# NumericalEarth/Breeze.jl

Measured on AMD Instinct MI355X. Metric: grid-cells advanced/sec (tendency+Poisson step), 512^3 anelastic, higher is better.
Workload: dtype f64

## Files before the change

breeze.jl_amd/csrc/bz_tendency5_kernels.h:

```cpp
#pragma once
#include "bz_internal.h"
#include "bz_weno.h"
#include "bz_tendency4_kernels.h"

typedef long long ix_t;
typedef unsigned ix32_t;

struct LevRow5 {
    double rho, rrho;
    double rho_f, rrho_f;
    double Ax, Ay, Vinv_c;
    double pi;
    double Vinv_f, T_r;
    double pad[6];
};
struct Lev5 {
    const LevRow5 *p;
#ifdef __HIPCC__
    __device__ __forceinline__ double at(int k, int f) const { return ((ColPtr::cptr)(const double *)p)[(long long)k * 16 + f]; }
    __device__ __forceinline__ double rho(int k) const { return at(k, 0); }
    __device__ __forceinline__ double rrho(int k) const { return at(k, 1); }
    __device__ __forceinline__ double rho_f(int k) const { return at(k, 2); }
    __device__ __forceinline__ double rrho_f(int k) const { return at(k, 3); }
    __device__ __forceinline__ double Ax(int k) const { return at(k, 4); }
    __device__ __forceinline__ double Ay(int k) const { return at(k, 5); }
    __device__ __forceinline__ double Vinv_c(int k) const { return at(k, 6); }
    __device__ __forceinline__ double pi(int k) const { return at(k, 7); }
    __device__ __forceinline__ double Vinv_f(int k) const { return at(k, 8); }
    __device__ __forceinline__ double T_r(int k) const { return at(k, 9); }
#endif
};
static_assert(sizeof(LevRow5) == 16 * sizeof(double), "LevRow5 is sixteen reals");

#define BZ_LEAN_WAVES (sizeof(double) == 8 ? 4 : 6)
#define BZ5_SCALAR_WAVES (sizeof(double) == 8 ? 4 : 6)
#define BZ6_W_WAVES 4
constexpr int BZ5_EB = 64;

struct Lean5 {
    const double *ru, *rv, *rw;
    const double *pa, *pb;
    double *out;
    double *oa, *ob;
    double *T;
    ColPtr pi_dry;
    const LevRow5 *lev;
    int mforce;
    double cor_f;
    ColPtr Fu, Fv;
    ColPtr Su, Sv;
    const double *vel, *bT, *bq;
    const int *qstate;
    int xcd;
    int by0, bys;
};
// ... 33 lines not shown
    const double th = bz_cdiv(rth, rho, rrho), q = bz_cdiv(rq, rho, rrho);
    if (pi_dry.p && __all(q == 0.0)) return pi_dry[k] * th;
    const double qd = 1.0 - q;
    const double cpm = qd * g.cpd + q * g.cpv;
    return bz_exner_factor(g, k, q, cpm) * th;
}

__device__ __forceinline__ double bz_temperature5r(const DevGrid &g, double rth, double rq, int k, double rho, double rrho, double pi)
{
    const double th = bz_cdiv(rth, rho, rrho), q = bz_cdiv(rq, rho, rrho);
    if (__all(q == 0.0)) return pi * th;
    const double qd = 1.0 - q;
    const double cpm = qd * g.cpd + q * g.cpv;
    return bz_exner_factor(g, k, q, cpm) * th;
}

template <bool WY> __device__ __forceinline__ int by5_face(const DevGrid &g, int j) { return WY ? bz_buffer_face(j, g.Ny) : 3; }
template <bool WY> __device__ __forceinline__ int by5_center(const DevGrid &g, int j) { return WY ? bz_buffer_center(j, g.Ny) : 3; }
template <bool WY>
__device__ __forceinline__ double bz_up5y(double m3, double m2, double m1, double p0, double p1, double p2, bool left, int B)
{
    if constexpr (WY) return bz_upB(m3, m2, m1, p0, p1, p2, left, B);
    else return bz_up5(m3, m2, m1, p0, p1, p2, left);
}
template <bool WY>
__device__ __forceinline__ double bz_symm4y(double qm2, double qm1, double q0, double qp1, int B)
{
    if constexpr (WY) return (B == 3) ? bz_symm4(qm2, qm1, q0, qp1) : bz_symm2(qm1, q0);
    else return bz_symm4(qm2, qm1, q0, qp1);
}

template <int TY, bool WY, bool DRYQ>
__device__ __forceinline__ void k5_scalar_pair_body(const DevGrid &g, const Lean5 &F, int kchunk, const RKEpilogue &E, double *Tp, double *FYp, int *ZF)
{
    constexpr bool Q = !DRYQ;
    constexpr int TR = TY + 6, TC = 72;
    constexpr int NHALO = TR * 70 - TY * 64;
    constexpr int NT = 64 * TY;
    constexpr int HPT = (NHALO + NT - 1) / NT;
    double(*T)[2][TR][TC] = (double(*)[2][TR][TC])Tp;
    double(*FY)[2][TY + 1][64] = (double(*)[2][TY + 1][64])FYp;
    constexpr bool ZS = Q;

    int bx, by, bz;
    bz_block5(F, bx, by, bz);
    const int tx = threadIdx.x, ty = threadIdx.y, t = ty * 64 + tx;
// ... 245 lines not shown
    }
}


template <bool DRYQ, bool GUARD>
__device__ __forceinline__ bool bz_lean_skip(const Lean5 &F)
{
    if constexpr (!GUARD) return false;
    const bool dry = F.qstate != nullptr && __builtin_amdgcn_readfirstlane(*F.qstate) == 1;
    return dry != DRYQ;
}
template <int TY, bool WY = false, bool DRYQ = false, bool GUARD = true>
__global__ __launch_bounds__(64 * TY) __attribute__((amdgpu_waves_per_eu(BZ5_SCALAR_WAVES, BZ5_SCALAR_WAVES))) void k5_scalar_pair(DevGrid g, Lean5 F, int kchunk, RKEpilogue E)
{
    constexpr int TR = TY + 6, TC = 72;
    __shared__ double T[2 * 2 * TR * TC];
    __shared__ double FY[2 * 2 * (TY + 1) * 64];
    __shared__ int ZF[3];
    if (bz_lean_skip<DRYQ, GUARD>(F)) return;
    k5_scalar_pair_body<TY, WY, DRYQ>(g, F, kchunk, E, T, FY, ZF);
}

template <int KIND>
__device__ __forceinline__ double flux_x_lean(const DevGrid &g, const Tend3Fields &F, const double *__restrict__ m, int i, int j, int k, int By = 3)
{
    const long long n = g.idx(i, j, k);
    const double a = (KIND == T3_V && By != 3) ? bz_symm2(g.Ax[k] * F.ru[n - g.Sx], g.Ax[k] * F.ru[n]) : adv_x<KIND>(g, F, n, k);
    const double rh = (KIND == T3_W) ? g.rho_f[k] : g.rho[k], rr = (KIND == T3_W) ? g.rrho_f[k] : g.rrho[k];
    if constexpr (KIND == T3_U)
        return a * bz_up5(bz_cdiv(m[n - 2], rh, rr), bz_cdiv(m[n - 1], rh, rr), bz_cdiv(m[n], rh, rr), bz_cdiv(m[n + 1], rh, rr),
                          bz_cdiv(m[n + 2], rh, rr), bz_cdiv(m[n + 3], rh, rr), a > 0.0);
    else
        return a * bz_up5(bz_cdiv(m[n - 3], rh, rr), bz_cdiv(m[n - 2], rh, rr), bz_cdiv(m[n - 1], rh, rr), bz_cdiv(m[n], rh, rr),
                          bz_cdiv(m[n + 1], rh, rr), bz_cdiv(m[n + 2], rh, rr), a > 0.0);
}


template <int TY, bool MF = false, bool WY = false, bool ST = false>
__global__ __launch_bounds__(64 * TY, BZ_LEAN_WAVES) void k6_u(DevGrid g, Lean5 L, int kchunk, RKEpilogue E)
{
    static_assert(!(ST && WY), "stored-velocity instantiations: periodic / slab rows");
    constexpr int TR = TY + 6, TC = 72, NT = 64 * TY;
    constexpr int NH1 = TR * 70 - TY * 64;
    constexpr int NH2 = 3 * (TY + 1) + 64 + 3 * TY;
    static_assert(NH1 <= NT && NH2 <= NT, "one frame cell of each kind per thread");
    __shared__ double U[2][TR][TC];
    __shared__ double RU[2][TY][TC];
    __shared__ double RV[2][TY + 1][TC];
    __shared__ double RW[2][TY][TC];
    __shared__ double FY[2][TY + 1][64];
    int bx, by, bz;
    bz_block5(L, bx, by, bz);
    const int tx = threadIdx.x, ty = threadIdx.y, t = ty * 64 + tx, tc = tx + 3;
    const int i0 = bx * 64, j0 = by * TY;
    const int i = i0 + tx, j = j0 + ty;
    const int ic = min(i, g.Nx + 2), jc = min(j, g.Ny + 2);
    const int ie = i0 - 1, le = 0;
    const int kbeg = bz * kchunk, kend = min(kbeg + kchunk, g.Nz);
    if (kbeg >= kend) return;
    const ix_t sz = (ix_t)g.Sxy;
    const bool store = (i < g.Nx) && (j < g.Ny);
    const double *__restrict__ ru = L.ru, *__restrict__ rv = L.rv, *__restrict__ rw = L.rw;
    const double *__restrict__ vel = ST ? L.vel : L.ru;
    Tend3Fields F;
    F.ru = L.ru; F.rv = L.rv; F.rw = L.rw; F.u = F.v = F.w = F.T = F.q = nullptr; F.c = ST ? L.vel : nullptr; F.G = L.out;
    ix_t n = (ix_t)g.idx(ic, jc, kbeg);
    const bool h1ok = t < NH1;
    int h1r = 0, h1c = 0;
    {
        const int h = h1ok ? t : 0;
        if (h < 6 * 70) { const int rr = h / 70; h1c = h - rr * 70; h1r = (rr < 3) ? rr : TY + rr; }
        else { const int hh = h - 6 * 70, rr = hh / 6, cc = hh - rr * 6; h1r = 3 + rr; h1c = (cc < 3) ? cc : 64 + cc; }
    }
    const ix_t h1n = (ix_t)g.idx(min(i0 - 3 + h1c, g.Nx + 2), min(j0 - 3 + h1r, g.Ny + 2), kbeg);
    const bool h1raw = h1ok && h1r >= 3 && h1r < TY + 3 && (h1c == 2 || h1c == 67 || h1c == 68);
    const bool h2ok = t < NH2;
    int h2sel = 0, h2r = 0, h2c = 0;
    {
        const int id = h2ok ? t : 0;
        if (id < 3 * (TY + 1)) { h2r = id / 3; const int cc = id - 3 * h2r; h2c = (cc < 2) ? 1 + cc : 67; }
        else if (id < 3 * (TY + 1) + 64) { h2r = TY; h2c = 3 + (id - 3 * (TY + 1)); }
        else { h2sel = 1; const int m = id - 3 * (TY + 1) - 64; h2r = m / 3; const int cc = m - 3 * h2r; h2c = (cc < 2) ? 1 + cc : 67; }
    }
    const double *__restrict__ h2src = h2sel ? rw : rv;
    const ix_t h2n = (ix_t)g.idx(min(i0 - 3 + h2c, g.Nx + 2), min(j0 + h2r, g.Ny + 2), kbeg) + (h2sel ? sz : (ix_t)0);

    double r[6];
#pragma unroll
    for (int s = 0; s < 6; ++s) r[s] = ST ? vel[n + s * sz - 3 * sz] : bz_cdiv(ru[n + s * sz - 3 * sz], g.rho[kbeg + s - 3], g.rrho[kbeg + s - 3]);
    double fz_lo = vflux<T3_U>(g, F, n, kbeg, r[0], r[1], r[2], r[3], r[4], r[5]);
    double q0 = ru[n], q1 = ru[n + sz], q2 = ru[n + 2 * sz];
    U[0][ty + 3][tc] = r[3];
    RU[0][ty][tc] = q0;
    RV[0][ty][tc] = rv[n];
    RW[0][ty][tc] = rw[n + sz];
    if (h1ok) {
        const double raw = (ST && !h1raw) ? 0.0 : ru[h1n];
        U[0][h1r][h1c] = ST ? vel[h1n] : bz_cdiv(raw, g.rho[kbeg], g.rrho[kbeg]);
        if (h1raw) RU[0][h1r - 3][h1c] = raw;
    }
    if (h2ok) { if (h2sel) RW[0][h2r][h2c] = h2src[h2n]; else RV[0][h2r][h2c] = h2src[h2n]; }
    double tcur_raw = ru[n + 3 * sz];
    double tcur_v = ST ? vel[n + 3 * sz] : 0.0;
    double u0cur = (E.mode == 2) ? E.u0[n] : 0.0;
    __syncthreads();

    double edge = 0.0;
    int buf = 0;
    for (int k = kbeg; k < kend; ++k, n += sz) {
        const ix_t lev1 = (ix_t)(k + 1 - kbeg) * sz;
        const double p_top = ST ? ru[n + sz] : ru[n + ((k + 4 <= g.Nz + g.Hz - 1) ? 4 * sz : 3 * sz)];
        const double p_topv = ST ? vel[n + ((k + 4 <= g.Nz + g.Hz - 1) ? 4 * sz : 3 * sz)] : 0.0;
        const double p_h1 = h1ok ? (ST ? vel : ru)[h1n + lev1] : 0.0;
        const double p_h1raw = (ST && h1raw) ? ru[h1n + lev1] : 0.0;
        const double p_h2 = h2ok ? h2src[h2n + lev1] : 0.0;
        const double p_rv = rv[n + sz], p_rw = rw[n + 2 * sz];
        const double p_u0 = (E.mode == 2) ? E.u0[n + sz] : 0.0;
        if (((k - kbeg) & (BZ5_EB - 1)) == 0) {
            const int kk = min(k + (tx & (BZ5_EB - 1)), kend - 1);
            edge = ST ? flux_x_at<T3_U>(g, F, ie, jc, kk) : flux_x_lean<T3_U>(g, F, ru, ie, jc, kk);
        }
        const int src = (k - kbeg) & (BZ5_EB - 1);
        const double Ax = g.Ax[k], Ay = g.Ay[k], Az = g.Az;
        const double c0 = r[3];
        const double(*Uk)[TC] = U[buf];
        const double *rur = RU[buf][ty] + tc, *ur = Uk[ty + 3] + tc;
        const double ax = bz_symm4(Ax * rur[-1], Ax * q0, Ax * rur[1], Ax * rur[2]);
        const double fx = ax * bz_up5(ur[-2], ur[-1], c0, ur[1], ur[2], ur[3], ax > 0.0);
        double nb = 0.0;
        if constexpr (!MF) {
            nb = bz_lane_up(fx);
            const double e = bz_lane_read(edge, src);
            if (tx == le) nb = e;
        }
        const double *rvr = RV[buf][ty] + tc;
        const double ay = bz_symm4(Ay * rvr[-2], Ay * rvr[-1], Ay * rvr[0], Ay * rvr[1]);
        const double fy = ay * bz_up5y<WY>(Uk[ty][tc], Uk[ty + 1][tc], Uk[ty + 2][tc], c0, Uk[ty + 4][tc], Uk[ty + 5][tc], ay > 0.0, by5_face<WY>(g, __builtin_amdgcn_readfirstlane(j)));
        FY[buf][ty][tx] = fy;
        if (ty == 0) {
            const double *rvt = RV[buf][TY] + tc;
            const double at = bz_symm4(Ay * rvt[-2], Ay * rvt[-1], Ay * rvt[0], Ay * rvt[1]);
            FY[buf][TY][tx] = at * bz_up5y<WY>(Uk[TY][tc], Uk[TY + 1][tc], Uk[TY + 2][tc], Uk[TY + 3][tc], Uk[TY + 4][tc], Uk[TY + 5][tc], at > 0.0,
                                               by5_face<WY>(g, j0 + TY));
        }
        const double tnew = ST ? tcur_v : bz_cdiv(tcur_raw, g.rho[k + 3], g.rrho[k + 3]);
        const double *rwr = RW[buf][ty] + tc;
        const double wt = bz_symm4(Az * rwr[-2], Az * rwr[-1], Az * rwr[0], Az * rwr[1]);
        const double fz_hi = wt * bz_upB(r[1], r[2], r[3], r[4], r[5], tnew, wt > 0.0, bz_buffer_face(k + 1, g.Nz));
        U[buf ^ 1][ty + 3][tc] = r[4];
        RU[buf ^ 1][ty][tc] = ST ? p_top : q1;
        RV[buf ^ 1][ty][tc] = p_rv;
        RW[buf ^ 1][ty][tc] = p_rw;
        if (h1ok) {
            U[buf ^ 1][h1r][h1c] = ST ? p_h1 : bz_cdiv(p_h1, g.rho[k + 1], g.rrho[k + 1]);
            if (h1raw) RU[buf ^ 1][h1r - 3][h1c] = ST ? p_h1raw : p_h1;
        }
        if (h2ok) { if (h2sel) RW[buf ^ 1][h2r][h2c] = p_h2; else RV[buf ^ 1][h2r][h2c] = p_h2; }
        __syncthreads();
        {
            if constexpr (MF) {
                nb = __shfl_up(fx, 1);
                const double e = __shfl(edge, src);
                if (tx == le) nb = e;
            }
            const double dx = fx - nb;
            const double dy = FY[buf][ty + 1][tx] - fy;
            double Gu = -(g.Vinv_c[k] * (dx + dy + (fz_hi - fz_lo)));
            if constexpr (MF) {
                if (L.mforce & 1) {
                    const double *rv0 = RV[buf][ty] + tc, *rv1 = RV[buf][ty + 1] + tc;
                    const double a = (rv0[-1] + rv1[-1]) / 2, b = (rv0[0] + rv1[0]) / 2;
                    Gu -= -L.cor_f * ((a + b) / 2);
                }
                if (L.mforce & (2 | 8)) {
                    const double rho = g.rho[k];
                    double tot = (L.mforce & 8) ? rho * L.Su[k] : 0.0;
                    if (L.mforce & 2) tot = (L.mforce & 8) ? tot + rho * L.Fu[k] : rho * L.Fu[k];
                    Gu += tot;
                }
            }
            if (store) L.out[n] = (ST && E.mode == 0) ? Gu : bz_rk_apply_pre(E.mode, E.dt, E.alpha, E.oma, u0cur, E.u0_out, Gu, q0, n);
        }
        fz_lo = fz_hi;
#pragma unroll
        for (int s = 0; s < 5; ++s) r[s] = r[s + 1];
        r[5] = tnew;
        if (ST) q0 = p_top;
        else { q0 = q1; q1 = q2; q2 = tcur_raw; tcur_raw = p_top; }
        u0cur = p_u0;
        if (ST) tcur_v = p_topv;
        buf ^= 1;
    }
}


template <int TY, bool MF = false, bool WY = false, bool ST = false>
__global__ __launch_bounds__(64 * TY, ((MF && WY) ? 4 : BZ_LEAN_WAVES)) void k6_v(DevGrid g, Lean5 L, int kchunk, RKEpilogue E)
{
    static_assert(!(ST && WY), "stored-velocity instantiations: periodic / slab rows");
    constexpr int RV = TY + 6, RM = TY + 4;
    constexpr int TC = 72;
    __shared__ double Tv[2][RV][TC];
    __shared__ double Tm[2][3][RM][64];
    __shared__ double FY[2][TY + 1][64];
    constexpr int NT = 64 * TY, NFR = 16 * 64, HPT = (NFR + NT - 1) / NT;
    int bx, by, bz;
    bz_block5(L, bx, by, bz);
    const int tx = threadIdx.x, ty = threadIdx.y, t = ty * 64 + tx, tc = tx + 3;
    const int i0 = bx * 64, j0 = by * TY;
    const int i = i0 + tx, j = j0 + ty;
    const int ic = min(i, g.Nx + 2), jc = min(j, g.Ny + 2);
    const int nact = min(64, g.Nx - i0);
    const int ie = i0 + nact, le = nact - 1;
    const int kbeg = bz * kchunk, kend = min(kbeg + kchunk, g.Nz);
    if (kbeg >= kend) return;
    const ix_t sz = (ix_t)g.Sxy;
    const bool store = (i < g.Nx) && (j < g.Ny) && !(WY && j == 0);
    const int ju = __builtin_amdgcn_readfirstlane(j);
    const int Bf = by5_face<WY>(g, ju), Bc = by5_center<WY>(g, ju), Bc0 = by5_center<WY>(g, j0 - 1);
    const double *__restrict__ ru = L.ru, *__restrict__ rv = L.rv, *__restrict__ rw = L.rw;
    const double *__restrict__ vel = ST ? L.vel : L.rv;
    Tend3Fields F;
    F.ru = L.ru; F.rv = L.rv; F.rw = L.rw; F.u = F.v = F.w = F.T = F.q = nullptr; F.c = ST ? L.vel : nullptr; F.G = L.out;
    const double Az = g.Az;
    ix_t n = (ix_t)g.idx(ic, jc, kbeg);

    bool hok[HPT];
    int hsel[HPT], hrow[HPT];
    ix_t hn[HPT];
    const double *hsrc[HPT];
#pragma unroll
    for (int q = 0; q < HPT; ++q) {
        const int h = t + q * NT;
        hok[q] = h < NFR;
        const int id = __builtin_amdgcn_readfirstlane(hok[q] ? (h >> 6) : 0);
        int sel, row, grow;
        if (id < 6) { sel = 0; row = (id < 3) ? id : TY + id; grow = j0 - 3 + row; }
        else if (id < 9) { sel = 1; const int m = id - 6; row = (m < 2) ? m : TY + 2; grow = j0 - 2 + row; }
        else if (id < 13) { sel = 2; const int m = id - 9; row = (m < 2) ? m : TY + m; grow = j0 - 2 + row; }
        else { sel = 3; const int m = id - 13; row = (m < 2) ? m : TY + 2; grow = j0 - 2 + row; }
        hsel[q] = sel; hrow[q] = row;
        hsrc[q] = (sel == 1) ? ru : (sel == 3) ? rw : (ST && sel == 0) ? vel : rv;
        hn[q] = (ix_t)g.idx(min(i0 + tx, g.Nx + 2), min(grow, g.Ny + 2), kbeg) + (sel == 3 ? sz : (ix_t)0);
    }
    auto frame_load = [&](int q, ix_t lev) -> double { return hsrc[q][hn[q] + lev]; };
    auto frame_store = [&](int b, int q, double raw, int klev) {
        if (hsel[q] == 0) Tv[b][hrow[q]][tc] = ST ? raw : bz_cdiv(raw, g.rho[klev], g.rrho[klev]);
        else Tm[b][hsel[q] - 1][hrow[q]][tx] = ((hsel[q] == 1) ? g.Ax[klev] : (hsel[q] == 2) ? g.Ay[klev] : Az) * raw;
    };

    const bool sok = t < 5 * TY;
    const int srow = sok ? t / 5 : 0, scc = sok ? t % 5 : 0, scol = (scc < 3) ? scc : 64 + scc;
    const ix_t sn = (ix_t)g.idx(min(i0 - 3 + scol, g.Nx + 2), min(j0 + srow, g.Ny + 2), kbeg);

    double r[6];
#pragma unroll
    for (int s = 0; s < 6; ++s) r[s] = ST ? vel[n + s * sz - 3 * sz] : bz_cdiv(rv[n + s * sz - 3 * sz], g.rho[kbeg + s - 3], g.rrho[kbeg + s - 3]);
    double fz_lo;
    if (WY && Bf != 3) {
        const double wt0 = bz_symm2(Az * rw[n - (ix_t)g.Sx], Az * rw[n]);
        fz_lo = wt0 * bz_upB(r[0], r[1], r[2], r[3], r[4], r[5], wt0 > 0.0, bz_buffer_face(kbeg, g.Nz));
    } else fz_lo = vflux<T3_V>(g, F, n, kbeg, r[0], r[1], r[2], r[3], r[4], r[5]);
    double q0 = rv[n], q1 = rv[n + sz], q2 = rv[n + 2 * sz];
    Tv[0][ty + 3][tc] = r[3];
    if (sok) Tv[0][srow + 3][scol] = ST ? vel[sn] : bz_cdiv(rv[sn], g.rho[kbeg], g.rrho[kbeg]);
    Tm[0][0][ty + 2][tx] = g.Ax[kbeg] * ru[n];
    Tm[0][1][ty + 2][tx] = g.Ay[kbeg] * q0;
    Tm[0][2][ty + 2][tx] = Az * rw[n + sz];
#pragma unroll
    for (int q = 0; q < HPT; ++q)
        if (hok[q]) frame_store(0, q, frame_load(q, 0), kbeg);
    __syncthreads();

    double tcur_raw = rv[n + 3 * sz];
    double tcur_v = ST ? vel[n + 3 * sz] : 0.0;
    double u0cur = (E.mode == 2) ? E.u0[n] : 0.0;
    double edge = 0.0;
    int buf = 0;
    for (int k = kbeg; k < kend; ++k, n += sz) {
        const ix_t lev = (ix_t)(k + 1 - kbeg) * sz;
        double hnext[HPT];
#pragma unroll
        for (int q = 0; q < HPT; ++q) hnext[q] = hok[q] ? frame_load(q, lev) : 0.0;
        const double p_side = sok ? (ST ? vel : rv)[sn + lev] : 0.0;
        const double p_top = ST ? rv[n + sz] : rv[n + ((k + 4 <= g.Nz + g.Hz - 1) ? 4 * sz : 3 * sz)];
        const double p_topv = ST ? vel[n + ((k + 4 <= g.Nz + g.Hz - 1) ? 4 * sz : 3 * sz)] : 0.0;
        const double p_u0 = (E.mode == 2) ? E.u0[n + sz] : 0.0;
        const double tnew_raw = tcur_raw, u0v = u0cur;
        const double ru_n = g.Ax[k + 1] * ru[n + sz], rw_n = Az * rw[n + 2 * sz];
        double cor_u = 0.0, cg1 = 0.0, cg3 = 0.0;
        if constexpr (MF) { if ((L.mforce & 1) && tx == 63) { const ix_t sy = (ix_t)g.Sx; cg1 = ru[n - sy + 1]; cg3 = ru[n + 1]; } }
        if (((k - kbeg) & (BZ5_EB - 1)) == 0) {
            const int kk = min(k + (tx & (BZ5_EB - 1)), kend - 1);
            edge = ST ? flux_x_at<T3_V>(g, F, ie, jc, kk) : flux_x_lean<T3_V>(g, F, rv, ie, jc, kk, Bf);
        }
        const int src = (k - kbeg) & (BZ5_EB - 1);
        const double rho = g.rho[k];
        const double c0 = r[3];
        const double(*V)[TC] = Tv[buf];
        const double *vrow = V[ty + 3] + tc;
        const double(*MU)[64] = Tm[buf][0];
        const double(*MV)[64] = Tm[buf][1];
        const double(*MW)[64] = Tm[buf][2];
        const double ut = bz_symm4y<WY>(MU[ty][tx], MU[ty + 1][tx], MU[ty + 2][tx], MU[ty + 3][tx], Bf);
        const double fx = ut * bz_up5(vrow[-3], vrow[-2], vrow[-1], c0, vrow[1], vrow[2], ut > 0.0);
        double nb = 0.0;
        if constexpr (!MF) {
            nb = bz_lane_down(fx);
            const double e = bz_lane_read(edge, src);
            if (tx == le) nb = e;
        }
        const double vt = (!WY || Bc == 3) ? bz_symm4(MV[ty + 1][tx], MV[ty + 2][tx], MV[ty + 3][tx], MV[ty + 4][tx]) : bz_symm2(MV[ty + 2][tx], MV[ty + 3][tx]);
        const double fy = vt * bz_up5y<WY>(V[ty + 1][tc], V[ty + 2][tc], c0, V[ty + 4][tc], V[ty + 5][tc], V[ty + 6][tc], vt > 0.0, Bc);
        FY[buf][ty + 1][tx] = fy;
        if (ty == 0) {
            const double vb = (!WY || Bc0 == 3) ? bz_symm4(MV[0][tx], MV[1][tx], MV[2][tx], MV[3][tx]) : bz_symm2(MV[1][tx], MV[2][tx]);
            FY[buf][0][tx] = vb * bz_up5y<WY>(V[0][tc], V[1][tc], V[2][tc], V[3][tc], V[4][tc], V[5][tc], vb > 0.0, Bc0);
        }
        const double tnew = ST ? tcur_v : bz_cdiv(tnew_raw, g.rho[k + 3], g.rrho[k + 3]);
        const double wt = bz_symm4y<WY>(MW[ty][tx], MW[ty + 1][tx], MW[ty + 2][tx], MW[ty + 3][tx], Bf);
        const double fz_hi = wt * bz_upB(r[1], r[2], r[3], r[4], r[5], tnew, wt > 0.0, bz_buffer_face(k + 1, g.Nz));
        if constexpr (MF) {
            if (L.mforce & 1) {
                const double Axk = g.Ax[k];
                const double l1 = MU[ty + 1][tx + 1], l3 = MU[ty + 2][tx + 1];
                const double c1 = (tx == 63) ? Axk * cg1 : l1, c3 = (tx == 63) ? Axk * cg3 : l3;
                cor_u = (((MU[ty + 1][tx] + c1) / 2 + (MU[ty + 2][tx] + c3) / 2) / 2) / Axk;
            }
        }
        Tv[buf ^ 1][ty + 3][tc] = r[4];
        if (sok) Tv[buf ^ 1][srow + 3][scol] = ST ? p_side : bz_cdiv(p_side, g.rho[k + 1], g.rrho[k + 1]);
        Tm[buf ^ 1][0][ty + 2][tx] = ru_n;
        Tm[buf ^ 1][1][ty + 2][tx] = g.Ay[k + 1] * (ST ? p_top : q1);
        Tm[buf ^ 1][2][ty + 2][tx] = rw_n;
#pragma unroll
        for (int q = 0; q < HPT; ++q)
            if (hok[q]) frame_store(buf ^ 1, q, hnext[q], k + 1);
        __syncthreads();
        {
            if constexpr (MF) {
                nb = __shfl_down(fx, 1);
                const double e = __shfl(edge, src);
                if (tx == le) nb = e;
            }
            const double dx = nb - fx;
            const double dy = fy - FY[buf][ty][tx];
            double Gv = -(g.Vinv_c[k] * (dx + dy + (fz_hi - fz_lo)));
            if constexpr (MF) {
                if (L.mforce & 1) Gv -= L.cor_f * cor_u;
                if (L.mforce & (4 | 16)) {
                    double tot = (L.mforce & 16) ? rho * L.Sv[k] : 0.0;
                    if (L.mforce & 4) tot = (L.mforce & 16) ? tot + rho * L.Fv[k] : rho * L.Fv[k];
                    Gv += tot;
                }
            }
            if (store) L.out[n] = (ST && E.mode == 0) ? Gv : bz_rk_apply_pre(E.mode, E.dt, E.alpha, E.oma, u0v, E.u0_out, Gv, q0, n);
            if constexpr (WY) {
                if (i < g.Nx && j == 0) L.out[n] = 0.0;
                if (i < g.Nx && j == g.Ny - 1) L.out[n + (ix_t)g.Sx] = 0.0;
            }
        }
        fz_lo = fz_hi;
        if (ST) q0 = p_top;
        else { q0 = q1; q1 = q2; q2 = tnew_raw; tcur_raw = p_top; }
        u0cur = p_u0;
        if (ST) tcur_v = p_topv;
#pragma unroll
        for (int s = 0; s < 5; ++s) r[s] = r[s + 1];
        r[5] = tnew;
        buf ^= 1;
// ... 185 lines not shown
```

breeze.jl_amd/csrc/bz_weno.h:

```cpp
#pragma once
#include <hip/hip_runtime.h>

#define BZ_WENO_EPS 1e-8

#ifndef BZ_WENO_ONE_DIVISION
#define BZ_WENO_ONE_DIVISION 1
#endif

__device__ __forceinline__ double bz_weno5_ref(double a, double b, double c, double d, double e)
{
    double b0 = c * (10.0 * c - 31.0 * d + 11.0 * e) + d * (25.0 * d - 19.0 * e) + e * (4.0 * e);
    double b1 = b * (4.0 * b - 13.0 * c + 5.0 * d) + c * (13.0 * c - 13.0 * d) + d * (4.0 * d);
    double b2 = a * (4.0 * a - 19.0 * b + 11.0 * c) + b * (25.0 * b - 31.0 * c) + c * (10.0 * c);
    double tau = fabs(b0 - b2);
    double r0 = tau / (b0 + BZ_WENO_EPS);
    double r1 = tau / (b1 + BZ_WENO_EPS);
    double r2 = tau / (b2 + BZ_WENO_EPS);
    double a0 = (3.0 / 10.0) * (1.0 + r0 * r0);
    double a1 = (3.0 / 5.0) * (1.0 + r1 * r1);
    double a2 = (1.0 / 10.0) * (1.0 + r2 * r2);
    double p0 = (1.0 / 3.0) * c + (5.0 / 6.0) * d - (1.0 / 6.0) * e;
    double p1 = -(1.0 / 6.0) * b + (5.0 / 6.0) * c + (1.0 / 3.0) * d;
    double p2 = (1.0 / 3.0) * a - (7.0 / 6.0) * b + (11.0 / 6.0) * c;
    return (a0 * p0 + a1 * p1 + a2 * p2) / (a0 + a1 + a2);
}

__device__ __forceinline__ double bz_weno5_fast(double a, double b, double c, double d, double e)
{
    const double D1 = b - a, D2 = c - b, D3 = d - c, D4 = e - d;
    const double S1 = D2 - D1, S2 = D3 - D2, S3 = D4 - D3;
    const double L2 = fma(3.0, D2, -D1), L1 = D2 + D3, L0 = fma(-3.0, D3, D4);
    const double E43 = (4.0 / 3.0) * BZ_WENO_EPS, C133 = 13.0 / 3.0;
    const double d2 = fma(L2, L2, fma(C133, S1 * S1, E43));
    const double d1 = fma(L1, L1, fma(C133, S2 * S2, E43));
    const double d0 = fma(L0, L0, fma(C133, S3 * S3, E43));
    const double tau = d0 - d2;
    const double t2 = tau * tau;
    const double s0 = d0 * d0, s1 = d1 * d1, s2 = d2 * d2;
    const double P0 = s1 * s2, P1 = s0 * s2, P2 = s0 * s1;
    const double Q = s0 * P0;
    const double a0 = fma(t2, P0, Q), a1 = fma(t2, P1, Q), a2 = fma(t2, P2, Q);
    const double e0 = fma(2.0, D3, -0.5 * D4);
    const double e1 = fma(2.0, D3, D2);
    const double e2 = fma(5.0 / 6.0, D2, -(1.0 / 3.0) * D1);
    const double num = fma(a2, e2, fma(a1, e1, a0 * e0));
    const double den = fma(3.0, a0, fma(6.0, a1, a2));
    double r = __builtin_amdgcn_rcp(den);
    r = fma(fma(-den, r, 1.0), r, r);
    r = fma(fma(-den, r, 1.0), r, r);
    return fma(num, r, c);
}

__device__ __forceinline__ double bz_weno5_diff(double a, double b, double c, double d, double e)
{
    const double D1 = b - a, D2 = c - b, D3 = d - c, D4 = e - d;
    const double S1 = D2 - D1, S2 = D3 - D2, S3 = D4 - D3;
    const double L2 = fma(3.0, D2, -D1), L1 = D2 + D3, L0 = fma(-3.0, D3, D4);
    const double E43 = (4.0 / 3.0) * BZ_WENO_EPS, C133 = 13.0 / 3.0;
    const double d2 = fma(L2, L2, fma(C133, S1 * S1, E43));
    const double d1 = fma(L1, L1, fma(C133, S2 * S2, E43));
    const double d0 = fma(L0, L0, fma(C133, S3 * S3, E43));
    const double tau = fabs(d0 - d2);
    const double r0 = tau * __builtin_amdgcn_rcp(d0), r1 = tau * __builtin_amdgcn_rcp(d1), r2 = tau * __builtin_amdgcn_rcp(d2);
    const double a0 = fma(r0, r0, 1.0), a1 = fma(r1, r1, 1.0), a2 = fma(r2, r2, 1.0);
    const double e0 = fma(2.0, D3, -0.5 * D4);
    const double e1 = fma(2.0, D3, D2);
    const double e2 = fma(5.0 / 6.0, D2, -(1.0 / 3.0) * D1);
    const double num = fma(a2, e2, fma(a1, e1, a0 * e0));
    const double den = fma(3.0, a0, fma(6.0, a1, a2));
    return fma(num, __builtin_amdgcn_rcp(den), c);
}

#ifndef BZ_WENO_FT2
#define BZ_WENO_FT2 0
// ... 26 lines not shown
    const double b1 = b * (4.0 * b - 13.0 * c + 5.0 * d) + c * (13.0 * c - 13.0 * d) + d * (4.0 * d);
    const double b2 = a * (4.0 * a - 19.0 * b + 11.0 * c) + b * (25.0 * b - 31.0 * c) + c * (10.0 * c);
    const double tau = fabs(b0 - b2);
    const double r0 = bz_newton_div(tau, b0 + BZ_WENO_EPS), r1 = bz_newton_div(tau, b1 + BZ_WENO_EPS), r2 = bz_newton_div(tau, b2 + BZ_WENO_EPS);
    const double a0 = (3.0 / 10.0) * (1.0 + r0 * r0), a1 = (3.0 / 5.0) * (1.0 + r1 * r1), a2 = (1.0 / 10.0) * (1.0 + r2 * r2);
    return (a0 * p0 + a1 * p1 + a2 * p2) / (a0 + a1 + a2);
#endif
}

__device__ __forceinline__ double bz_weno5(double a, double b, double c, double d, double e)
{
#if BZ_WENO_FT2
    return bz_weno5_ft2(a, b, c, d, e);
#endif
#if BZ_WENO_ONE_DIVISION == 2
    return bz_weno5_diff(a, b, c, d, e);
#elif BZ_WENO_ONE_DIVISION
    return bz_weno5_fast(a, b, c, d, e);
#else
    return bz_weno5_ref(a, b, c, d, e);
#endif
}

template <int NR>
__device__ __forceinline__ double bz_recip(double x)
{
    double r = __builtin_amdgcn_rcp(x);
    if (sizeof(double) == 8) {
#pragma unroll
        for (int it = 0; it < NR; ++it) r = fma(fma(-x, r, 1.0), r, r);
    }
    return r;
}

__device__ __forceinline__ double bz_weno3(double a, double b, double c)
{
    double p0 = 0.5 * b + 0.5 * c;
    double p1 = -0.5 * a + 1.5 * b;
#if BZ_WENO_FT2 == 2
    {
        const float af = (float)a, bf = (float)b, cf = (float)c;
        const float b0 = (cf - bf) * (cf - bf), b1 = (bf - af) * (bf - af);
        const float tau = fabsf(b0 - b1);
        const float r0 = tau / (b0 + 1e-8f), r1 = tau / (b1 + 1e-8f);
        const float a0 = (2.0f / 3.0f) * (1.0f + r0 * r0), a1 = (1.0f / 3.0f) * (1.0f + r1 * r1);
        const float sum = a0 + a1;
// ... 18 lines not shown
template <class R>
__device__ __forceinline__ R bz_sel(unsigned long long m, R a, R b)
{
    if constexpr (sizeof(R) == 8) {
        const int alo = __double2loint(a), ahi = __double2hiint(a), blo = __double2loint(b), bhi = __double2hiint(b);
        int lo, hi;
        asm("v_cndmask_b32_e64 %0, %1, %2, %3" : "=v"(lo) : "v"(blo), "v"(alo), "s"(m));
        asm("v_cndmask_b32_e64 %0, %1, %2, %3" : "=v"(hi) : "v"(bhi), "v"(ahi), "s"(m));
        return __hiloint2double(hi, lo);
    } else {
        const int ai = __float_as_int(a), bi = __float_as_int(b);
        int r;
        asm("v_cndmask_b32_e64 %0, %1, %2, %3" : "=v"(r) : "v"(bi), "v"(ai), "s"(m));
        return __int_as_float(r);
    }
}
__device__ __forceinline__ unsigned long long bz_lanes(bool p) { return __builtin_amdgcn_ballot_w64(p); }
constexpr bool BZ_UPWIND_UNIFORM = sizeof(double) == 8;

#ifdef BZ_CENTERED2
__device__ __forceinline__ double bz_up5(double, double, double m1, double p0, double, double, bool) { return 0.5 * (m1 + p0); }
__device__ __forceinline__ double bz_up3(double, double m1, double p0, double, bool) { return 0.5 * (m1 + p0); }
__device__ __forceinline__ double bz_upB(double, double, double m1, double p0, double, double, bool, int) { return 0.5 * (m1 + p0); }
#else
__device__ __forceinline__ double bz_up5(double m3, double m2, double m1, double p0, double p1,
                                         double p2, bool left)
{
    const unsigned long long m = bz_lanes(left);
    if constexpr (BZ_UPWIND_UNIFORM) {
    if (m == bz_lanes(true)) return bz_weno5(m3, m2, m1, p0, p1);
    if (m == 0ull) return bz_weno5(p2, p1, p0, m1, m2);
    }
    double a = bz_sel(m, m3, p2);
    double b = bz_sel(m, m2, p1);
    double c = bz_sel(m, m1, p0);
    double d = bz_sel(m, p0, m1);
    double e = bz_sel(m, p1, m2);
    return bz_weno5(a, b, c, d, e);
}
__device__ __forceinline__ double bz_up3(double m2, double m1, double p0, double p1, bool left)
{
    const unsigned long long m = bz_lanes(left);
    double a = bz_sel(m, m2, p1);
    double b = bz_sel(m, m1, p0);
    double c = bz_sel(m, p0, m1);
    return bz_weno3(a, b, c);
}
__device__ __forceinline__ double bz_upB(double m3, double m2, double m1, double p0, double p1,
                                         double p2, bool left, int B)
{
    if (B == 3) return bz_up5(m3, m2, m1, p0, p1, p2, left);
    if (B == 2) return bz_up3(m2, m1, p0, p1, left);
    return bz_sel(bz_lanes(left), m1, p0);
}
#endif

__device__ __forceinline__ int bz_buffer_face(int idx, int N)
{
    if (idx >= 3 && idx <= N - 3) return 3;
    if (idx >= 2 && idx <= N - 2) return 2;
    return 1;
}
__device__ __forceinline__ int bz_buffer_center(int idx, int N)
{
    if (idx >= 2 && idx <= N - 3) return 3;
    if (idx >= 1 && idx <= N - 2) return 2;
    return 1;
}

__device__ __forceinline__ double bz_symm4(double qm2, double qm1, double q0, double qp1)
{
#ifdef BZ_CENTERED2
    return 0.5 * (qm1 + q0);
#else
    return (7.0 / 12.0) * (qm1 + q0) - (1.0 / 12.0) * (qm2 + qp1);
#endif
// ... 3 lines not shown
```

Measured before the change: 4.183 billion.

## Pin WENO constants in VGPRs and read level coefficients from packed row table

WENO5 stencil constants are now passed as a struct. In the non-forcing, non-wall, non-stored u/v kernel instantiations they are pinned in vector registers with empty asm, so the f64 FMAs stop rematerialising 64-bit literal constants on every call. The u and v momentum kernels also read rho, rrho, Ax, Ay and Vinv_c from the packed 16-double LevRow5 table (one row per level) instead of separate DevGrid arrays, except in the stored-velocity path. The pinned constants cost extra VGPRs and may lower occupancy under the launch bounds, and the x-edge flux now recomputes its advecting velocity inline.

```diff
diff --git a/breeze.jl_amd/csrc/bz_tendency5_kernels.h b/breeze.jl_amd/csrc/bz_tendency5_kernels.h
--- a/breeze.jl_amd/csrc/bz_tendency5_kernels.h
+++ b/breeze.jl_amd/csrc/bz_tendency5_kernels.h
@@ -31,6 +31,17 @@
 #endif
 };
 static_assert(sizeof(LevRow5) == 16 * sizeof(double), "LevRow5 is sixteen reals");
+template <bool ST> struct LevSrc5 {
+    const DevGrid &g;
+    const Lev5 LV;
+#ifdef __HIPCC__
+    __device__ __forceinline__ double rho(int k) const { if constexpr (ST) return g.rho[k]; else return LV.rho(k); }
+    __device__ __forceinline__ double rrho(int k) const { if constexpr (ST) return g.rrho[k]; else return LV.rrho(k); }
+    __device__ __forceinline__ double Ax(int k) const { if constexpr (ST) return g.Ax[k]; else return LV.Ax(k); }
+    __device__ __forceinline__ double Ay(int k) const { if constexpr (ST) return g.Ay[k]; else return LV.Ay(k); }
+    __device__ __forceinline__ double Vinv_c(int k) const { if constexpr (ST) return g.Vinv_c[k]; else return LV.Vinv_c(k); }
+#endif
+};
 
 #define BZ_LEAN_WAVES (sizeof(double) == 8 ? 4 : 6)
 #define BZ5_SCALAR_WAVES (sizeof(double) == 8 ? 4 : 6)
@@ -110,6 +121,12 @@
 {
     if constexpr (WY) return bz_upB(m3, m2, m1, p0, p1, p2, left, B);
     else return bz_up5(m3, m2, m1, p0, p1, p2, left);
+}
+template <bool WY>
+__device__ __forceinline__ double bz_up5y(double m3, double m2, double m1, double p0, double p1, double p2, bool left, int B, const BzWeno5K &K)
+{
+    if constexpr (WY) return bz_upB(m3, m2, m1, p0, p1, p2, left, B, K);
+    else return bz_up5(m3, m2, m1, p0, p1, p2, left, K);
 }
 template <bool WY>
 __device__ __forceinline__ double bz_symm4y(double qm2, double qm1, double q0, double qp1, int B)
@@ -401,11 +418,21 @@
 }
 
 template <int KIND>
-__device__ __forceinline__ double flux_x_lean(const DevGrid &g, const Tend3Fields &F, const double *__restrict__ m, int i, int j, int k, int By = 3)
+__device__ __forceinline__ double flux_x_lean(const DevGrid &g, const Tend3Fields &F, const double *__restrict__ m, int i, int j, int k, int By = 3,
+                                              const Lev5 LV = Lev5{nullptr})
 {
     const long long n = g.idx(i, j, k);
-    const double a = (KIND == T3_V && By != 3) ? bz_symm2(g.Ax[k] * F.ru[n - g.Sx], g.Ax[k] * F.ru[n]) : adv_x<KIND>(g, F, n, k);
-    const double rh = (KIND == T3_W) ? g.rho_f[k] : g.rho[k], rr = (KIND == T3_W) ? g.rrho_f[k] : g.rrho[k];
+    double a, rh, rr;
+    if constexpr (KIND == T3_W) {
+        a = adv_x<KIND>(g, F, n, k);
+        rh = g.rho_f[k]; rr = g.rrho_f[k];
+    } else {
+        const double A = LV.Ax(k);
+        const long long sy = g.Sx;
+        if constexpr (KIND == T3_U) a = bz_symm4(A * F.ru[n - 1], A * F.ru[n], A * F.ru[n + 1], A * F.ru[n + 2]);
+        else a = (By != 3) ? bz_symm2(A * F.ru[n - sy], A * F.ru[n]) : bz_symm4(A * F.ru[n - 2 * sy], A * F.ru[n - sy], A * F.ru[n], A * F.ru[n + sy]);
+        rh = LV.rho(k); rr = LV.rrho(k);
+    }
     if constexpr (KIND == T3_U)
         return a * bz_up5(bz_cdiv(m[n - 2], rh, rr), bz_cdiv(m[n - 1], rh, rr), bz_cdiv(m[n], rh, rr), bz_cdiv(m[n + 1], rh, rr),
                           bz_cdiv(m[n + 2], rh, rr), bz_cdiv(m[n + 3], rh, rr), a > 0.0);
@@ -441,6 +468,7 @@
     const bool store = (i < g.Nx) && (j < g.Ny);
     const double *__restrict__ ru = L.ru, *__restrict__ rv = L.rv, *__restrict__ rw = L.rw;
     const double *__restrict__ vel = ST ? L.vel : L.ru;
+    const LevSrc5<ST> C{g, Lev5{L.lev}};
     Tend3Fields F;
     F.ru = L.ru; F.rv = L.rv; F.rw = L.rw; F.u = F.v = F.w = F.T = F.q = nullptr; F.c = ST ? L.vel : nullptr; F.G = L.out;
     ix_t n = (ix_t)g.idx(ic, jc, kbeg);
@@ -466,7 +494,7 @@
 
     double r[6];
 #pragma unroll
-    for (int s = 0; s < 6; ++s) r[s] = ST ? vel[n + s * sz - 3 * sz] : bz_cdiv(ru[n + s * sz - 3 * sz], g.rho[kbeg + s - 3], g.rrho[kbeg + s - 3]);
+    for (int s = 0; s < 6; ++s) r[s] = ST ? vel[n + s * sz - 3 * sz] : bz_cdiv(ru[n + s * sz - 3 * sz], C.rho(kbeg + s - 3), C.rrho(kbeg + s - 3));
     double fz_lo = vflux<T3_U>(g, F, n, kbeg, r[0], r[1], r[2], r[3], r[4], r[5]);
     double q0 = ru[n], q1 = ru[n + sz], q2 = ru[n + 2 * sz];
     U[0][ty + 3][tc] = r[3];
@@ -475,7 +503,7 @@
     RW[0][ty][tc] = rw[n + sz];
     if (h1ok) {
         const double raw = (ST && !h1raw) ? 0.0 : ru[h1n];
-        U[0][h1r][h1c] = ST ? vel[h1n] : bz_cdiv(raw, g.rho[kbeg], g.rrho[kbeg]);
+        U[0][h1r][h1c] = ST ? vel[h1n] : bz_cdiv(raw, C.rho(kbeg), C.rrho(kbeg));
         if (h1raw) RU[0][h1r - 3][h1c] = raw;
     }
     if (h2ok) { if (h2sel) RW[0][h2r][h2c] = h2src[h2n]; else RV[0][h2r][h2c] = h2src[h2n]; }
@@ -486,6 +514,7 @@
 
     double edge = 0.0;
     int buf = 0;
+    const BzWeno5K K = bz_weno5_k_regs<!MF && !WY && !ST>();
     for (int k = kbeg; k < kend; ++k, n += sz) {
         const ix_t lev1 = (ix_t)(k + 1 - kbeg) * sz;
         const double p_top = ST ? ru[n + sz] : ru[n + ((k + 4 <= g.Nz + g.Hz - 1) ? 4 * sz : 3 * sz)];
@@ -497,15 +526,15 @@
         const double p_u0 = (E.mode == 2) ? E.u0[n + sz] : 0.0;
         if (((k - kbeg) & (BZ5_EB - 1)) == 0) {
             const int kk = min(k + (tx & (BZ5_EB - 1)), kend - 1);
-            edge = ST ? flux_x_at<T3_U>(g, F, ie, jc, kk) : flux_x_lean<T3_U>(g, F, ru, ie, jc, kk);
+            edge = ST ? flux_x_at<T3_U>(g, F, ie, jc, kk) : flux_x_lean<T3_U>(g, F, ru, ie, jc, kk, 3, C.LV);
         }
         const int src = (k - kbeg) & (BZ5_EB - 1);
-        const double Ax = g.Ax[k], Ay = g.Ay[k], Az = g.Az;
+        const double Ax = C.Ax(k), Ay = C.Ay(k), Az = g.Az;
         const double c0 = r[3];
         const double(*Uk)[TC] = U[buf];
         const double *rur = RU[buf][ty] + tc, *ur = Uk[ty + 3] + tc;
         const double ax = bz_symm4(Ax * rur[-1], Ax * q0, Ax * rur[1], Ax * rur[2]);
-        const double fx = ax * bz_up5(ur[-2], ur[-1], c0, ur[1], ur[2], ur[3], ax > 0.0);
+        const double fx = ax * bz_up5(ur[-2], ur[-1], c0, ur[1], ur[2], ur[3], ax > 0.0, K);
         double nb = 0.0;
         if constexpr (!MF) {
             nb = bz_lane_up(fx);
@@ -514,24 +543,24 @@
         }
         const double *rvr = RV[buf][ty] + tc;
         const double ay = bz_symm4(Ay * rvr[-2], Ay * rvr[-1], Ay * rvr[0], Ay * rvr[1]);
-        const double fy = ay * bz_up5y<WY>(Uk[ty][tc], Uk[ty + 1][tc], Uk[ty + 2][tc], c0, Uk[ty + 4][tc], Uk[ty + 5][tc], ay > 0.0, by5_face<WY>(g, __builtin_amdgcn_readfirstlane(j)));
+        const double fy = ay * bz_up5y<WY>(Uk[ty][tc], Uk[ty + 1][tc], Uk[ty + 2][tc], c0, Uk[ty + 4][tc], Uk[ty + 5][tc], ay > 0.0, by5_face<WY>(g, __builtin_amdgcn_readfirstlane(j)), K);
         FY[buf][ty][tx] = fy;
         if (ty == 0) {
             const double *rvt = RV[buf][TY] + tc;
             const double at = bz_symm4(Ay * rvt[-2], Ay * rvt[-1], Ay * rvt[0], Ay * rvt[1]);
             FY[buf][TY][tx] = at * bz_up5y<WY>(Uk[TY][tc], Uk[TY + 1][tc], Uk[TY + 2][tc], Uk[TY + 3][tc], Uk[TY + 4][tc], Uk[TY + 5][tc], at > 0.0,
-                                               by5_face<WY>(g, j0 + TY));
-        }
-        const double tnew = ST ? tcur_v : bz_cdiv(tcur_raw, g.rho[k + 3], g.rrho[k + 3]);
+                                               by5_face<WY>(g, j0 + TY), K);
+        }
+        const double tnew = ST ? tcur_v : bz_cdiv(tcur_raw, C.rho(k + 3), C.rrho(k + 3));
         const double *rwr = RW[buf][ty] + tc;
         const double wt = bz_symm4(Az * rwr[-2], Az * rwr[-1], Az * rwr[0], Az * rwr[1]);
-        const double fz_hi = wt * bz_upB(r[1], r[2], r[3], r[4], r[5], tnew, wt > 0.0, bz_buffer_face(k + 1, g.Nz));
+        const double fz_hi = wt * bz_upB(r[1], r[2], r[3], r[4], r[5], tnew, wt > 0.0, bz_buffer_face(k + 1, g.Nz), K);
         U[buf ^ 1][ty + 3][tc] = r[4];
         RU[buf ^ 1][ty][tc] = ST ? p_top : q1;
         RV[buf ^ 1][ty][tc] = p_rv;
         RW[buf ^ 1][ty][tc] = p_rw;
         if (h1ok) {
-            U[buf ^ 1][h1r][h1c] = ST ? p_h1 : bz_cdiv(p_h1, g.rho[k + 1], g.rrho[k + 1]);
+            U[buf ^ 1][h1r][h1c] = ST ? p_h1 : bz_cdiv(p_h1, C.rho(k + 1), C.rrho(k + 1));
             if (h1raw) RU[buf ^ 1][h1r - 3][h1c] = ST ? p_h1raw : p_h1;
         }
         if (h2ok) { if (h2sel) RW[buf ^ 1][h2r][h2c] = p_h2; else RV[buf ^ 1][h2r][h2c] = p_h2; }
@@ -544,7 +573,7 @@
             }
             const double dx = fx - nb;
             const double dy = FY[buf][ty + 1][tx] - fy;
-            double Gu = -(g.Vinv_c[k] * (dx + dy + (fz_hi - fz_lo)));
+            double Gu = -(C.Vinv_c(k) * (dx + dy + (fz_hi - fz_lo)));
             if constexpr (MF) {
                 if (L.mforce & 1) {
                     const double *rv0 = RV[buf][ty] + tc, *rv1 = RV[buf][ty + 1] + tc;
@@ -552,7 +581,7 @@
                     Gu -= -L.cor_f * ((a + b) / 2);
                 }
                 if (L.mforce & (2 | 8)) {
-                    const double rho = g.rho[k];
+                    const double rho = C.rho(k);
                     double tot = (L.mforce & 8) ? rho * L.Su[k] : 0.0;
                     if (L.mforce & 2) tot = (L.mforce & 8) ? tot + rho * L.Fu[k] : rho * L.Fu[k];
                     Gu += tot;
@@ -599,6 +628,7 @@
     const int Bf = by5_face<WY>(g, ju), Bc = by5_center<WY>(g, ju), Bc0 = by5_center<WY>(g, j0 - 1);
     const double *__restrict__ ru = L.ru, *__restrict__ rv = L.rv, *__restrict__ rw = L.rw;
     const double *__restrict__ vel = ST ? L.vel : L.rv;
+    const LevSrc5<ST> C{g, Lev5{L.lev}};
     Tend3Fields F;
     F.ru = L.ru; F.rv = L.rv; F.rw = L.rw; F.u = F.v = F.w = F.T = F.q = nullptr; F.c = ST ? L.vel : nullptr; F.G = L.out;
     const double Az = g.Az;
@@ -624,8 +654,8 @@
     }
     auto frame_load = [&](int q, ix_t lev) -> double { return hsrc[q][hn[q] + lev]; };
     auto frame_store = [&](int b, int q, double raw, int klev) {
-        if (hsel[q] == 0) Tv[b][hrow[q]][tc] = ST ? raw : bz_cdiv(raw, g.rho[klev], g.rrho[klev]);
-        else Tm[b][hsel[q] - 1][hrow[q]][tx] = ((hsel[q] == 1) ? g.Ax[klev] : (hsel[q] == 2) ? g.Ay[klev] : Az) * raw;
+        if (hsel[q] == 0) Tv[b][hrow[q]][tc] = ST ? raw : bz_cdiv(raw, C.rho(klev), C.rrho(klev));
+        else Tm[b][hsel[q] - 1][hrow[q]][tx] = ((hsel[q] == 1) ? C.Ax(klev) : (hsel[q] == 2) ? C.Ay(klev) : Az) * raw;
     };
 
     const bool sok = t < 5 * TY;
@@ -634,7 +664,7 @@
 
     double r[6];
 #pragma unroll
-    for (int s = 0; s < 6; ++s) r[s] = ST ? vel[n + s * sz - 3 * sz] : bz_cdiv(rv[n + s * sz - 3 * sz], g.rho[kbeg + s - 3], g.rrho[kbeg + s - 3]);
+    for (int s = 0; s < 6; ++s) r[s] = ST ? vel[n + s * sz - 3 * sz] : bz_cdiv(rv[n + s * sz - 3 * sz], C.rho(kbeg + s - 3), C.rrho(kbeg + s - 3));
     double fz_lo;
     if (WY && Bf != 3) {
         const double wt0 = bz_symm2(Az * rw[n - (ix_t)g.Sx], Az * rw[n]);
@@ -642,9 +672,9 @@
     } else fz_lo = vflux<T3_V>(g, F, n, kbeg, r[0], r[1], r[2], r[3], r[4], r[5]);
     double q0 = rv[n], q1 = rv[n + sz], q2 = rv[n + 2 * sz];
     Tv[0][ty + 3][tc] = r[3];
-    if (sok) Tv[0][srow + 3][scol] = ST ? vel[sn] : bz_cdiv(rv[sn], g.rho[kbeg], g.rrho[kbeg]);
-    Tm[0][0][ty + 2][tx] = g.Ax[kbeg] * ru[n];
-    Tm[0][1][ty + 2][tx] = g.Ay[kbeg] * q0;
+    if (sok) Tv[0][srow + 3][scol] = ST ? vel[sn] : bz_cdiv(rv[sn], C.rho(kbeg), C.rrho(kbeg));
+    Tm[0][0][ty + 2][tx] = C.Ax(kbeg) * ru[n];
+    Tm[0][1][ty + 2][tx] = C.Ay(kbeg) * q0;
     Tm[0][2][ty + 2][tx] = Az * rw[n + sz];
 #pragma unroll
     for (int q = 0; q < HPT; ++q)
@@ -656,6 +686,7 @@
     double u0cur = (E.mode == 2) ? E.u0[n] : 0.0;
     double edge = 0.0;
     int buf = 0;
+    const BzWeno5K K = bz_weno5_k_regs<TY == 16 && !MF && !WY && !ST>();
     for (int k = kbeg; k < kend; ++k, n += sz) {
         const ix_t lev = (ix_t)(k + 1 - kbeg) * sz;
         double hnext[HPT];
@@ -666,15 +697,15 @@
         const double p_topv = ST ? vel[n + ((k + 4 <= g.Nz + g.Hz - 1) ? 4 * sz : 3 * sz)] : 0.0;
         const double p_u0 = (E.mode == 2) ? E.u0[n + sz] : 0.0;
         const double tnew_raw = tcur_raw, u0v = u0cur;
-        const double ru_n = g.Ax[k + 1] * ru[n + sz], rw_n = Az * rw[n + 2 * sz];
+        const double ru_n = C.Ax(k + 1) * ru[n + sz], rw_n = Az * rw[n + 2 * sz];
         double cor_u = 0.0, cg1 = 0.0, cg3 = 0.0;
         if constexpr (MF) { if ((L.mforce & 1) && tx == 63) { const ix_t sy = (ix_t)g.Sx; cg1 = ru[n - sy + 1]; cg3 = ru[n + 1]; } }
         if (((k - kbeg) & (BZ5_EB - 1)) == 0) {
             const int kk = min(k + (tx & (BZ5_EB - 1)), kend - 1);
-            edge = ST ? flux_x_at<T3_V>(g, F, ie, jc, kk) : flux_x_lean<T3_V>(g, F, rv, ie, jc, kk, Bf);
+            edge = ST ? flux_x_at<T3_V>(g, F, ie, jc, kk) : flux_x_lean<T3_V>(g, F, rv, ie, jc, kk, Bf, C.LV);
         }
         const int src = (k - kbeg) & (BZ5_EB - 1);
-        const double rho = g.rho[k];
+        const double rho = C.rho(k);
         const double c0 = r[3];
         const double(*V)[TC] = Tv[buf];
         const double *vrow = V[ty + 3] + tc;
@@ -682,7 +713,7 @@
         const double(*MV)[64] = Tm[buf][1];
         const double(*MW)[64] = Tm[buf][2];
         const double ut = bz_symm4y<WY>(MU[ty][tx], MU[ty + 1][tx], MU[ty + 2][tx], MU[ty + 3][tx], Bf);
-        const double fx = ut * bz_up5(vrow[-3], vrow[-2], vrow[-1], c0, vrow[1], vrow[2], ut > 0.0);
+        const double fx = ut * bz_up5(vrow[-3], vrow[-2], vrow[-1], c0, vrow[1], vrow[2], ut > 0.0, K);
         double nb = 0.0;
         if constexpr (!MF) {
             nb = bz_lane_down(fx);
@@ -690,27 +721,27 @@
             if (tx == le) nb = e;
         }
         const double vt = (!WY || Bc == 3) ? bz_symm4(MV[ty + 1][tx], MV[ty + 2][tx], MV[ty + 3][tx], MV[ty + 4][tx]) : bz_symm2(MV[ty + 2][tx], MV[ty + 3][tx]);
-        const double fy = vt * bz_up5y<WY>(V[ty + 1][tc], V[ty + 2][tc], c0, V[ty + 4][tc], V[ty + 5][tc], V[ty + 6][tc], vt > 0.0, Bc);
+        const double fy = vt * bz_up5y<WY>(V[ty + 1][tc], V[ty + 2][tc], c0, V[ty + 4][tc], V[ty + 5][tc], V[ty + 6][tc], vt > 0.0, Bc, K);
         FY[buf][ty + 1][tx] = fy;
         if (ty == 0) {
             const double vb = (!WY || Bc0 == 3) ? bz_symm4(MV[0][tx], MV[1][tx], MV[2][tx], MV[3][tx]) : bz_symm2(MV[1][tx], MV[2][tx]);
-            FY[buf][0][tx] = vb * bz_up5y<WY>(V[0][tc], V[1][tc], V[2][tc], V[3][tc], V[4][tc], V[5][tc], vb > 0.0, Bc0);
-        }
-        const double tnew = ST ? tcur_v : bz_cdiv(tnew_raw, g.rho[k + 3], g.rrho[k + 3]);
+            FY[buf][0][tx] = vb * bz_up5y<WY>(V[0][tc], V[1][tc], V[2][tc], V[3][tc], V[4][tc], V[5][tc], vb > 0.0, Bc0, K);
+        }
+        const double tnew = ST ? tcur_v : bz_cdiv(tnew_raw, C.rho(k + 3), C.rrho(k + 3));
         const double wt = bz_symm4y<WY>(MW[ty][tx], MW[ty + 1][tx], MW[ty + 2][tx], MW[ty + 3][tx], Bf);
-        const double fz_hi = wt * bz_upB(r[1], r[2], r[3], r[4], r[5], tnew, wt > 0.0, bz_buffer_face(k + 1, g.Nz));
+        const double fz_hi = wt * bz_upB(r[1], r[2], r[3], r[4], r[5], tnew, wt > 0.0, bz_buffer_face(k + 1, g.Nz), K);
         if constexpr (MF) {
             if (L.mforce & 1) {
-                const double Axk = g.Ax[k];
+                const double Axk = C.Ax(k);
                 const double l1 = MU[ty + 1][tx + 1], l3 = MU[ty + 2][tx + 1];
                 const double c1 = (tx == 63) ? Axk * cg1 : l1, c3 = (tx == 63) ? Axk * cg3 : l3;
                 cor_u = (((MU[ty + 1][tx] + c1) / 2 + (MU[ty + 2][tx] + c3) / 2) / 2) / Axk;
             }
         }
         Tv[buf ^ 1][ty + 3][tc] = r[4];
-        if (sok) Tv[buf ^ 1][srow + 3][scol] = ST ? p_side : bz_cdiv(p_side, g.rho[k + 1], g.rrho[k + 1]);
+        if (sok) Tv[buf ^ 1][srow + 3][scol] = ST ? p_side : bz_cdiv(p_side, C.rho(k + 1), C.rrho(k + 1));
         Tm[buf ^ 1][0][ty + 2][tx] = ru_n;
-        Tm[buf ^ 1][1][ty + 2][tx] = g.Ay[k + 1] * (ST ? p_top : q1);
+        Tm[buf ^ 1][1][ty + 2][tx] = C.Ay(k + 1) * (ST ? p_top : q1);
         Tm[buf ^ 1][2][ty + 2][tx] = rw_n;
 #pragma unroll
         for (int q = 0; q < HPT; ++q)
@@ -724,7 +755,7 @@
             }
             const double dx = nb - fx;
             const double dy = fy - FY[buf][ty][tx];
-            double Gv = -(g.Vinv_c[k] * (dx + dy + (fz_hi - fz_lo)));
+            double Gv = -(C.Vinv_c(k) * (dx + dy + (fz_hi - fz_lo)));
             if constexpr (MF) {
                 if (L.mforce & 1) Gv -= L.cor_f * cor_u;
                 if (L.mforce & (4 | 16)) {
diff --git a/breeze.jl_amd/csrc/bz_weno.h b/breeze.jl_amd/csrc/bz_weno.h
--- a/breeze.jl_amd/csrc/bz_weno.h
+++ b/breeze.jl_amd/csrc/bz_weno.h
@@ -25,12 +25,30 @@
     return (a0 * p0 + a1 * p1 + a2 * p2) / (a0 + a1 + a2);
 }
 
-__device__ __forceinline__ double bz_weno5_fast(double a, double b, double c, double d, double e)
+struct BzWeno5K {
+    double c3, c6, c133, e43, c56, cm13;
+};
+__device__ __forceinline__ BzWeno5K bz_weno5_k() { return BzWeno5K{3.0, 6.0, 13.0 / 3.0, (4.0 / 3.0) * BZ_WENO_EPS, 5.0 / 6.0, -(1.0 / 3.0)}; }
+template <bool PIN>
+__device__ __forceinline__ BzWeno5K bz_weno5_k_regs()
+{
+    BzWeno5K K = bz_weno5_k();
+    if constexpr (PIN) {
+        asm("" : "+v"(K.c3));
+        asm("" : "+v"(K.c6));
+        asm("" : "+v"(K.c133));
+        asm("" : "+v"(K.e43));
+        asm("" : "+v"(K.c56));
+        asm("" : "+v"(K.cm13));
+    }
+    return K;
+}
+__device__ __forceinline__ double bz_weno5_fast(double a, double b, double c, double d, double e, const BzWeno5K &K)
 {
     const double D1 = b - a, D2 = c - b, D3 = d - c, D4 = e - d;
     const double S1 = D2 - D1, S2 = D3 - D2, S3 = D4 - D3;
-    const double L2 = fma(3.0, D2, -D1), L1 = D2 + D3, L0 = fma(-3.0, D3, D4);
-    const double E43 = (4.0 / 3.0) * BZ_WENO_EPS, C133 = 13.0 / 3.0;
+    const double L2 = fma(K.c3, D2, -D1), L1 = D2 + D3, L0 = fma(-K.c3, D3, D4);
+    const double E43 = K.e43, C133 = K.c133;
     const double d2 = fma(L2, L2, fma(C133, S1 * S1, E43));
     const double d1 = fma(L1, L1, fma(C133, S2 * S2, E43));
     const double d0 = fma(L0, L0, fma(C133, S3 * S3, E43));
@@ -42,14 +60,15 @@
     const double a0 = fma(t2, P0, Q), a1 = fma(t2, P1, Q), a2 = fma(t2, P2, Q);
     const double e0 = fma(2.0, D3, -0.5 * D4);
     const double e1 = fma(2.0, D3, D2);
-    const double e2 = fma(5.0 / 6.0, D2, -(1.0 / 3.0) * D1);
+    const double e2 = fma(K.c56, D2, K.cm13 * D1);
     const double num = fma(a2, e2, fma(a1, e1, a0 * e0));
-    const double den = fma(3.0, a0, fma(6.0, a1, a2));
+    const double den = fma(K.c3, a0, fma(K.c6, a1, a2));
     double r = __builtin_amdgcn_rcp(den);
     r = fma(fma(-den, r, 1.0), r, r);
     r = fma(fma(-den, r, 1.0), r, r);
     return fma(num, r, c);
 }
+__device__ __forceinline__ double bz_weno5_fast(double a, double b, double c, double d, double e) { return bz_weno5_fast(a, b, c, d, e, bz_weno5_k()); }
 
 __device__ __forceinline__ double bz_weno5_diff(double a, double b, double c, double d, double e)
 {
@@ -122,6 +141,15 @@
 #endif
 }
 
+__device__ __forceinline__ double bz_weno5(double a, double b, double c, double d, double e, const BzWeno5K &K)
+{
+#if BZ_WENO_ONE_DIVISION == 1 && !BZ_WENO_FT2
+    return bz_weno5_fast(a, b, c, d, e, K);
+#else
+    return bz_weno5(a, b, c, d, e);
+#endif
+}
+
 template <int NR>
 __device__ __forceinline__ double bz_recip(double x)
 {
@@ -186,21 +214,27 @@
 __device__ __forceinline__ double bz_up5(double, double, double m1, double p0, double, double, bool) { return 0.5 * (m1 + p0); }
 __device__ __forceinline__ double bz_up3(double, double m1, double p0, double, bool) { return 0.5 * (m1 + p0); }
 __device__ __forceinline__ double bz_upB(double, double, double m1, double p0, double, double, bool, int) { return 0.5 * (m1 + p0); }
+__device__ __forceinline__ double bz_up5(double, double, double m1, double p0, double, double, bool, const BzWeno5K &) { return 0.5 * (m1 + p0); }
+__device__ __forceinline__ double bz_upB(double, double, double m1, double p0, double, double, bool, int, const BzWeno5K &) { return 0.5 * (m1 + p0); }
 #else
 __device__ __forceinline__ double bz_up5(double m3, double m2, double m1, double p0, double p1,
-                                         double p2, bool left)
+                                         double p2, bool left, const BzWeno5K &K)
 {
     const unsigned long long m = bz_lanes(left);
     if constexpr (BZ_UPWIND_UNIFORM) {
-    if (m == bz_lanes(true)) return bz_weno5(m3, m2, m1, p0, p1);
-    if (m == 0ull) return bz_weno5(p2, p1, p0, m1, m2);
+    if (m == bz_lanes(true)) return bz_weno5(m3, m2, m1, p0, p1, K);
+    if (m == 0ull) return bz_weno5(p2, p1, p0, m1, m2, K);
     }
     double a = bz_sel(m, m3, p2);
     double b = bz_sel(m, m2, p1);
     double c = bz_sel(m, m1, p0);
     double d = bz_sel(m, p0, m1);
     double e = bz_sel(m, p1, m2);
-    return bz_weno5(a, b, c, d, e);
+    return bz_weno5(a, b, c, d, e, K);
+}
+__device__ __forceinline__ double bz_up5(double m3, double m2, double m1, double p0, double p1, double p2, bool left)
+{
+    return bz_up5(m3, m2, m1, p0, p1, p2, left, bz_weno5_k());
 }
 __device__ __forceinline__ double bz_up3(double m2, double m1, double p0, double p1, bool left)
 {
@@ -211,11 +245,15 @@
     return bz_weno3(a, b, c);
 }
 __device__ __forceinline__ double bz_upB(double m3, double m2, double m1, double p0, double p1,
-                                         double p2, bool left, int B)
-{
-    if (B == 3) return bz_up5(m3, m2, m1, p0, p1, p2, left);
+                                         double p2, bool left, int B, const BzWeno5K &K)
+{
+    if (B == 3) return bz_up5(m3, m2, m1, p0, p1, p2, left, K);
     if (B == 2) return bz_up3(m2, m1, p0, p1, left);
     return bz_sel(bz_lanes(left), m1, p0);
+}
+__device__ __forceinline__ double bz_upB(double m3, double m2, double m1, double p0, double p1, double p2, bool left, int B)
+{
+    return bz_upB(m3, m2, m1, p0, p1, p2, left, B, bz_weno5_k());
 }
 #endif
 
```

Result: no change. 4.196 billion (median of 6 runs) (+0.3%).
